# tsinghua-fib-lab/PIML

Measured on AMD Instinct MI355X. Metric: agent-pair force evals/sec + simulated steps/sec, 4096-agent GC scene, higher is better.
Workload: dtype f32

## Files before the change

include/piml_hip_tuning.h:

```cpp
#ifndef PIML_HIP_TUNING_H
#define PIML_HIP_TUNING_H

#include "piml_hip.h"

#ifdef __cplusplus
extern "C" {
#endif

int piml_timer_create(void** event);
int piml_timer_record(void* event, void* stream);
int piml_timer_elapsed_ms(void* start, void* stop, float* ms);
int piml_timer_destroy(void* event);

int piml_trace_begin(void);
int piml_trace_mark(const char* name, void* stream);
int piml_trace_end(char* names, int names_cap, float* us, int us_cap);

int piml_probe_arith(const float* rx, const float* ry, const float* hx, const float* hy,
                     float* dist, float* cosv, int n, void* stream);

long long piml_encoder_split_tiles(long long tiles);
long long piml_encoder_split_tiles_train(long long tiles);
int piml_encoder_products(int split_bf16);
int piml_rowdecoder_products(int split_bf16);
int piml_encoder_dw2(int layer_split);
int piml_encoder_fused_bwd(int on);
int piml_encoder_sums_bwd(int form);
int piml_pinnsf_streams_init(void);

#ifdef __cplusplus
}
#endif
#endif
```

piml_amd/_lib.py:

```python
import ctypes
import os

import torch

_HERE = os.path.dirname(os.path.abspath(__file__))
LIB_PATH = os.environ.get('PIML_LIB') or os.path.join(_HERE, 'libpiml_hip.so')
ABI_VERSION = 35

_lib = None

_i, _f, _p, _z = ctypes.c_int, ctypes.c_float, ctypes.c_void_p, ctypes.c_size_t
_ll = ctypes.c_longlong
_d = ctypes.c_double


class EncoderBranch(ctypes.Structure):
    _fields_ = [('x', _p), ('rows', _ll), ('in_dim', _i), ('k', _i),
                ('w1', _p), ('b1', _p), ('w2', _p), ('b2', _p), ('w3', _p), ('b3', _p),
                ('scale', _f), ('h1', _p), ('h2', _p), ('msgs', _p), ('g_pooled', _p), ('g_msgs', _p),
                ('g2', _p), ('g1', _p), ('g_x', _p), ('partials', _p), ('grads', _p), ('packed', _p), ('relu_mask', _p),
                ('keep_bits', _p), ('drop_state', _p), ('drop_p', _f), ('sum_a', _p), ('sum_b', _p)]


class DecoderBranch(ctypes.Structure):
# ... 98 lines not shown
    'piml_pinnsf_epilogue_ksum_bwd': [_p, _p, _z, _f, _i, _i, _p, _p, _p, _p],
    'piml_pinnsf_epilogue_agentnorm_fwd': [_p, _p, _p, _i, _i, _f, _p, _p],
    'piml_pinnsf_epilogue_ksum_agentnorm_fwd': [_p, _i, _p, _i, _p, _i, _i, _f, _p, _p],
    'piml_pinnsf_epilogue_agentnorm_bwd': [_p, _p, _i, _i, _f, _p, _p],
    'piml_self_features_fwd': [_p, _i, _p, _p, _z, _p, _p],
    'piml_self_features_bwd': [_p, _z, _p, _p, _p, _p],
    'piml_colsum_blocks': [_z, _i],
    'piml_act_bwd_colsum': [_p, _p, _z, _i, _p, _p, _p, _p],
    'piml_sum_leading': [_p, _i, _z, _p, _p],
    'piml_act_bwd_colsum_stage1': [_p, _p, _z, _i, _p, _p, _p, _p],
    'piml_layer_reduce': [_p, _i, _z, _p, _p, _i, _i, _p, _p],
    'piml_scale_ksum_fwd': [_p, _p, _z, _i, _i, _f, _p, _p, _p, _p],
    'piml_ksum_blocks': [_z, _i],
    'piml_scale_ksum_bwd': [_p, _p, _z, _i, _i, _f, _p, _p, _p, _p],
    'piml_dropout_keep_bits': [_p, _ll, _i, _f, _i, _p, _p],
    'piml_timer_create': [ctypes.POINTER(_p)],
    'piml_timer_record': [_p, _p],
    'piml_timer_elapsed_ms': [_p, _p, ctypes.POINTER(_f)],
    'piml_timer_destroy': [_p],
    'piml_trace_begin': [],
    'piml_trace_mark': [ctypes.c_char_p, _p],
    'piml_trace_end': [ctypes.c_char_p, _i, ctypes.POINTER(_f), _i],
    'piml_probe_arith': [_p, _p, _p, _p, _p, _p, _i, _p],
    'piml_encoder_partial_floats': [],
    'piml_encoder_pack_floats': [],
    'piml_encoder_split_tiles': [_ll],
    'piml_encoder_split_tiles_train': [_ll],
    'piml_multi_copy': [ctypes.POINTER(_p), ctypes.POINTER(_p), ctypes.POINTER(_z), _i, _p],
    'piml_rollout_prologue': [_p] * 8 + [_i] * 4 + [_p] * 11 + [_p],
    'piml_rollout_losses_blocks': [_i, _i],
    'piml_rollout_losses': [_p, _p, _ll, _p, _p, _p, _p, _p, _i, _i, _i, _f, _p, _p, _p, _p, _p, _p, _p],
    'piml_rollout_losses_bwd': [_p, _p, _p, _p, _p, _p, _ll, _p, _p],
    'piml_rollout_losses_frames': [_p, _p, _ll, _p, _p, ctypes.POINTER(_p), _i, _p, _i, _i, _i, _f, _f, _f, _p, _p, _p, _p, _p, _p, _p],
    'piml_rollout_losses_frames_bwd': [_p, _p, _p, _p, _f, _f, _p, _p, _p, _ll, _p, _p],
    'piml_collision_pred_loss_blocks': [_ll, _i],
    'piml_collision_pred_loss': [ctypes.POINTER(_p), ctypes.POINTER(_p), _i, _ll, _i, _i, _p, _i, _i, _f, _p, _p, _p, _p, _p],
    'piml_collision_pred_loss_bwd': [_p, _p, _ll, _p, _p],
    'piml_adam_tickets': [],
    'piml_adam_step': [ctypes.POINTER(_p)] * 5 + [ctypes.POINTER(_ll), _i, ctypes.c_double, ctypes.c_double, ctypes.c_double, ctypes.c_double, ctypes.c_double, _p, _p],
    'piml_pointwise_losses_blocks': [_ll, _ll, _i],
    'piml_pointwise_losses': [_p, _p, _ll, _ll, _p, _ll, _f, _p, _i, _p, _p, _p, _p, _p],
    'piml_p2p_alloc': [_z, ctypes.POINTER(_p)],
    'piml_p2p_free': [_p],
    'piml_p2p_export': [_p, _p],
    'piml_p2p_open': [_p, ctypes.POINTER(_p)],
    'piml_p2p_close': [_p],
    'piml_p2p_copy': [_p, _p, _z, _p],
    'piml_allgather_state_p2p': [_p, _z, _i, _i, ctypes.POINTER(_p), ctypes.POINTER(_p), ctypes.c_uint, ctypes.c_uint, _p, _p],
    'piml_encoder_products': [_i],
    'piml_rowdecoder_products': [_i],
    'piml_encoder_dw2': [_i],
    'piml_encoder_fused_bwd': [_i],
    'piml_encoder_sums_bwd': [_i],
    'piml_encoder_pack': [ctypes.POINTER(EncoderBranch), _i, _p],
    'piml_encoder_workgroups': [ctypes.POINTER(EncoderBranch), _i, ctypes.POINTER(_i)],
    'piml_encoder_fwd': [ctypes.POINTER(EncoderBranch), _i, _p],
    'piml_encoder_fwd_packed': [ctypes.POINTER(EncoderBranch), _i, _p],
    'piml_encoder_bwd': [ctypes.POINTER(EncoderBranch), _i, _p],
    'piml_encoder_bwd_acc': [ctypes.POINTER(EncoderBranch), _i, _i, _p],
    'piml_encoder_ksum': [_p, _ll, _i, _p, _p],
    'piml_decoder_pack_floats': [],
    'piml_decoder_partial_floats': [],
    'piml_decoder_workgroups': [_ll],
    'piml_decoder_fwd': [ctypes.POINTER(DecoderBranch), _i, _p, _f, _p, _p],
    'piml_decoder_bwd': [ctypes.POINTER(DecoderBranch), _i, _p, _p, _f, _p, _p],
    'piml_rowdecoder_slots': [_ll],
    'piml_rowdecoder_fwd': [ctypes.POINTER(DecoderBranch), _i, _p],
    'piml_rowdecoder_fwd_packed': [ctypes.POINTER(DecoderBranch), _i, _p],
    'piml_rowdecoder_bwd': [ctypes.POINTER(DecoderBranch), _i, _p],
    'piml_rowdecoder_bwd_acc': [ctypes.POINTER(DecoderBranch), _i, _i, _p],
    'piml_collision_head_pack_floats': [],
    'piml_collision_head_fwd': [_p, _ll, _p, _p, _p, _p, _p, _p, _p],
    'piml_head64_partial_floats': [],
    'piml_head64_slots': [_ll],
    'piml_head64_fwd': [ctypes.POINTER(Head64), _p],
    'piml_head64_bwd': [ctypes.POINTER(Head64), _p],
    'piml_head64_bwd_acc': [ctypes.POINTER(Head64), _i, _p],
    'piml_corrector_partial_floats': [_i],
    'piml_corrector_slots': [_i, _ll, _i],
    'piml_corrector_fwd': [ctypes.POINTER(Corrector), _p],
    'piml_corrector_bwd': [ctypes.POINTER(Corrector), _i, _p],
    'piml_pinnsf_pool_h2_ok': [ctypes.POINTER(EncoderBranch), _i],
    'piml_pinnsf_pool_train_ok': [ctypes.POINTER(EncoderBranch), _i],
    'piml_pinnsf_pool_msgs_ok': [ctypes.POINTER(EncoderBranch), _i],
    'piml_pinnsf_streams_init': [],
    'piml_pinnsf_pack_flush': [],
    'piml_pinnsf_slot_sums_flush': [],
    'piml_pinnsf_pack': [ctypes.POINTER(EncoderBranch), ctypes.POINTER(DecoderBranch), _i, ctypes.POINTER(CollisionHead),
                         _i, _p],
    'piml_pinnsf_fwd': [ctypes.POINTER(EncoderBranch), ctypes.POINTER(DecoderBranch), _i, ctypes.POINTER(CollisionHead),
                        _p, _f, _p, _i, _p],
    'piml_pinnsf_bwd': [ctypes.POINTER(EncoderBranch), ctypes.POINTER(DecoderBranch), _i, _p, _p, _f, _p, _i, _p],
    'piml_comm_available': [],
    'piml_comm_unique_id': [_p],
    'piml_comm_init': [ctypes.POINTER(_p), _i, _i, _p],
    'piml_comm_destroy': [_p],
    'piml_allgather_state': [_p, _p, _z, _p, _p],
    'piml_reducescatter_grad': [_p, _p, _p, _z, _p],
    'piml_allreduce_sum': [_p, _p, _z, _p],
    'piml_relfeat_fwd_self': [_p, _p, _p, _p, _i, _p, _p, _p, _i, _i, _i, _i, _i, _i, _i, _f, _f, _f, _f, _p, _p, _p, _p, _p, _p, _p],
    'piml_relfeat_bwd_self': [_p, _p, _p, _p, _p, _p, _i, _p, _i, _i, _i, _i, _i, _i, _p, _p, _p, _p],
    'piml_relfeat_fwd_tick': [_p, _p, _p, _p, _i, _p, _p, _i, _i, _i, _i, _i, _i, _i, _f, _f, _f, _f,
                              _p, _p, _p, _i, _p, _p, _p, _p],
    'piml_relfeat_self_fwd': [_p, _p, _p, _p, _i, _i, _i, _i, _i, _i, _f, _f, _f, _f, _p, _p, _p, _p, _p, _p, _p],
    'piml_relfeat_self_fwd_part': [_i, _p, _p, _p, _p, _i, _i, _i, _i, _i, _i, _f, _f, _f, _f, _p, _p, _p, _p, _p, _p, _p],
    'piml_relfeat_self_bwd': [_p, _p, _p, _p, _p, _p, _p, _i, _i, _i, _i, _i, _p, _p, _p, _p],
# ... 157 lines not shown
```

piml_amd/csrc/decoder.hip:

```cpp
#include <cstdlib>
#include <type_traits>

#include "common.hpp"
#include "pack.hpp"
#include "reduce.hpp"
#include "stages.hpp"
#include "x3.hpp"
#include "../../include/piml_hip.h"

namespace piml {

typedef float f32x16 __attribute__((ext_vector_type(16)));

constexpr int DEC_SLAB = 32;

struct DecArgs {
    piml_decoder_branch br[2];
    int nbr;
    const float* self_features;
    float tau;
    float* acc;
    const float* g_pred;
    float* g_self;
    int wg_split;
    int pool_h2;
};

#ifdef PIML_DEC_STAMPS
__device__ unsigned long long g_dec_stamps[1024 * 16];
#define DEC_STAMP(i, wait)                                                                         \
    do {                                                                                           \
        __builtin_amdgcn_sched_barrier(0);                                                         \
        if (wait) asm volatile("s_waitcnt vmcnt(0) lgkmcnt(0)" ::: "memory");                      \
        if (threadIdx.x == 0 && blockIdx.x < 1024) g_dec_stamps[blockIdx.x * 16 + (i)] = __builtin_amdgcn_s_memtime(); \
        __builtin_amdgcn_sched_barrier(0);                                                         \
    } while (0)
#else
#define DEC_STAMP(i, wait)
#endif

__device__ __forceinline__ f32x16 dmfma(float a, float b, f32x16 c) {
    return __builtin_amdgcn_mfma_f32_32x32x2f32(a, b, c, 0, 0, 0);
}
__device__ __forceinline__ int dfeat0(int blk, int q, int h) { return 32 * blk + 8 * q + 4 * h; }

__global__ __launch_bounds__(256) void dec_pack_kernel(DecArgs A) {
    const int b = blockIdx.y;
    const piml_decoder_branch J = b ? A.br[1] : A.br[0];
    const int e = blockIdx.x * 256 + threadIdx.x;
    if (e < DEC_PACK) J.packed[e] = dec_pack_value(J, e);
}

__device__ __forceinline__ void dec_pool_body(const piml_decoder_branch& J, long long bx) {
    const long long t = bx * 256 + threadIdx.x;
    if (t >= J.agents * (DH / 4)) return;
    const long long a = t / (DH / 4);
    const int c = (int)(t % (DH / 4));
    const float4* p = reinterpret_cast<const float4*>(J.msgs) + a * J.k * (DH / 4) + c;
    float4 s = make_float4(0.f, 0.f, 0.f, 0.f);
    for (int i = 0; i < J.k; ++i) {
        const float4 v = p[(size_t)i * (DH / 4)];
        s.x += v.x; s.y += v.y; s.z += v.z; s.w += v.w;
    }
    reinterpret_cast<float4*>(J.pooled)[t] = s;
}

__global__ __launch_bounds__(256) void dec_pool_kernel(DecArgs A) {
    dec_pool_body(blockIdx.y ? A.br[1] : A.br[0], blockIdx.x);
}

constexpr int POOL_ROWS = 10;

template <bool POOL, bool SPLIT = false, bool ROWS = false>
__device__ __forceinline__ void dec_fwd_body(const DecArgs& A, long long tile, int split_branch = 0) {
    constexpr int NB = SPLIT ? 1 : 2;
    __shared__ float part1[NB][2][2][16][64];
    __shared__ float part2[NB][2][2][16][64];
    __shared__ float part3[NB][2][2][32];
    __shared__ float poolx[POOL ? NB : 1][POOL ? 4 : 1][POOL ? 16 : 1][64];
    const int lane = threadIdx.x & 63, wave = uniform((int)(threadIdx.x >> 6));
    const int j = lane & 31, h = lane >> 5;
    const int b = SPLIT ? split_branch : wave >> 2, ob = (wave >> 1) & 1, kh = wave & 1;
    const int bi = SPLIT ? 0 : b;
    const bool active = b < A.nbr;
    const piml_decoder_branch J = b ? A.br[1] : A.br[0];
    const long long agent = tile * 32 + j;
    const bool valid = active && agent < J.agents;
    const float4* PK = reinterpret_cast<const float4*>(J.packed);
    const float* bias = J.packed + DP_B;
    float4 w2f[4], w3f[4], w1f[2][4], b2v[4];
// ... 167 lines not shown
#pragma unroll
            for (int q = 0; q < 4; ++q)
                *reinterpret_cast<float4*>(o + dfeat0(kh, q, h)) = make_float4(y[4 * q], y[4 * q + 1], y[4 * q + 2], y[4 * q + 3]);
        }
        f32x16 a3;
#pragma unroll
        for (int r = 0; r < 16; ++r) a3[r] = 0.f;
        if (h == 0 && kh == 0) { a3[0] = b3x; a3[1] = b3y; }
#pragma unroll
        for (int q = 0; q < 4; ++q) {
            const float4 w = w3f[q];
            a3 = dmfma(w.x, y[4 * q + 0], a3);
            a3 = dmfma(w.y, y[4 * q + 1], a3);
            a3 = dmfma(w.z, y[4 * q + 2], a3);
            a3 = dmfma(w.w, y[4 * q + 3], a3);
        }
        if (h == 0) { part3[bi][kh][0][j] = a3[0]; part3[bi][kh][1][j] = a3[1]; }
        if (SPLIT && !POOL && !ROWS) DEC_STAMP(7, true);
    }
    __syncthreads();
    if (SPLIT && !POOL && !ROWS) DEC_STAMP(8, false);
    if (ROWS) {
        if ((wave & 3) == 0 && h == 0 && agent < J.agents)
            reinterpret_cast<float2*>(J.pred)[agent] = make_float2(part3[0][0][0][j] + part3[0][1][0][j],
                                                                   part3[0][0][1][j] + part3[0][1][1][j]);
        return;
    }
    if (wave == 0 && h == 0 && agent < A.br[0].agents) {
        float ax = part3[0][0][0][j] + part3[0][1][0][j], ay = part3[0][0][1][j] + part3[0][1][1][j];
        if (A.self_features && b == 0) {
            const float dx = sfv[0], dy = sfv[1], vx = sfv[2], vy = sfv[3], v0 = sfv[4];
            float t = norm2(dx, dy);
            t = (t == 0.f) ? t + 0.1f : t;
            ax += (v0 * (dx / t) - vx) / A.tau;
            ay += (v0 * (dy / t) - vy) / A.tau;
        }
        if (SPLIT) {
            if (A.nbr > 1) {
                atomicAdd(A.acc + 2 * agent, ax);
                atomicAdd(A.acc + 2 * agent + 1, ay);
            } else {
                reinterpret_cast<float2*>(A.acc)[agent] = make_float2(ax, ay);
            }
        } else {
            if (A.nbr > 1) { ax += part3[1][0][0][j] + part3[1][1][0][j]; ay += part3[1][0][1][j] + part3[1][1][1][j]; }
            reinterpret_cast<float2*>(A.acc)[agent] = make_float2(ax, ay);
        }
    }
    if (SPLIT && !POOL && !ROWS) DEC_STAMP(9, true);
}

__global__ __launch_bounds__(512) void dec_fwd_kernel(DecArgs A) { dec_fwd_body<false>(A, blockIdx.x); }

template <bool ROWS = false, bool SPLIT = false>
__device__ __forceinline__ void dec_bwd_dx_body(const DecArgs& A, long long tile, int rows_branch = 0, float* keep_g2 = nullptr,
                                                float* keep_g1 = nullptr) {
    constexpr int NB = (ROWS || SPLIT) ? 1 : 2;
    __shared__ float part[NB][2][2][16][64];
    const int lane = threadIdx.x & 63, wave = uniform((int)(threadIdx.x >> 6));
    const int j = lane & 31, h = lane >> 5;
    const int b = (ROWS || SPLIT) ? rows_branch : wave >> 2, ob = (wave >> 1) & 1, kh = wave & 1, blk = wave & 3;
    const int bi = (ROWS || SPLIT) ? 0 : b;
    const bool active = b < A.nbr;
    const piml_decoder_branch J = b ? A.br[1] : A.br[0];
    const long long agent = tile * 32 + j;
    const bool valid = active && agent < J.agents;
    const float4* PK = reinterpret_cast<const float4*>(J.packed);
    float2 gp = make_float2(0.f, 0.f);
    float4 hv[2][4], t1f[8];
    float sfv[5] = {0.f, 0.f, 0.f, 0.f, 0.f};
    if (active) {
        gp = reinterpret_cast<const float2*>(ROWS ? J.g_pred_rows : A.g_pred)[valid ? agent : 0];
        if (!valid) gp = make_float2(0.f, 0.f);
        float4 gd2[4];
        if (ROWS && J.g_d2) {
#pragma unroll
            for (int q = 0; q < 4; ++q) gd2[q] = *reinterpret_cast<const float4*>(J.g_d2 + (valid ? agent : 0) * DD + dfeat0(kh, q, h));
        }
        if (!ROWS && wave == 0 && b == 0 && A.g_self && A.self_features) {
            const float* sp = A.self_features + (valid ? agent : 0) * 7;
            sfv[0] = sp[0]; sfv[1] = sp[1]; sfv[4] = sp[6];
        }
        const float bg = h ? gp.y : gp.x;
        const float* hp = J.h1 + (valid ? agent : 0) * DD;
#pragma unroll
        for (int o2 = 0; o2 < 2; ++o2)
#pragma unroll
            for (int q = 0; q < 4; ++q) hv[o2][q] = *reinterpret_cast<const float4*>(hp + dfeat0(o2, q, h));
        const float t3f = J.packed[DP_T3 + 64 * kh + lane];
        float4 t2f[4];
#pragma unroll
        for (int q = 0; q < 4; ++q) t2f[q] = PK[DP_T2 / 4 + (ob * 8 + kh * 4 + q) * 64 + lane];
#pragma unroll
        for (int t = 0; t < 8; ++t) t1f[t] = PK[((!ROWS && A.pool_h2 == 2) ? DP_T1F : DP_T1) / 4 + (blk * 8 + t) * 64 + lane];
        __builtin_amdgcn_sched_barrier(0);
        if (SPLIT) { DEC_STAMP(1, false); DEC_STAMP(2, true); }
        f32x16 g2, g1;
#pragma unroll
        for (int r = 0; r < 16; ++r) { g2[r] = 0.f; g1[r] = 0.f; }
        g2 = dmfma(t3f, bg, g2);
        if (ROWS && J.g_d2) {
#pragma unroll
            for (int q = 0; q < 4; ++q) {
                g2[4 * q] += valid ? gd2[q].x : 0.f; g2[4 * q + 1] += valid ? gd2[q].y : 0.f;
                g2[4 * q + 2] += valid ? gd2[q].z : 0.f; g2[4 * q + 3] += valid ? gd2[q].w : 0.f;
            }
        }
        if (SPLIT && keep_g2) {
            if (ob == 0) {
#pragma unroll
                for (int q = 0; q < 4; ++q)
                    *reinterpret_cast<float4*>(keep_g2 + j * DD + dfeat0(kh, q, h)) =
                        valid ? make_float4(g2[4 * q], g2[4 * q + 1], g2[4 * q + 2], g2[4 * q + 3]) : make_float4(0.f, 0.f, 0.f, 0.f);
            }
        } else if (ob == 0 && valid) {
            float* o = J.g_pre2 + agent * DD;
#pragma unroll
            for (int q = 0; q < 4; ++q)
                *reinterpret_cast<float4*>(o + dfeat0(kh, q, h)) = make_float4(g2[4 * q], g2[4 * q + 1], g2[4 * q + 2], g2[4 * q + 3]);
        }
#pragma unroll
        for (int q = 0; q < 4; ++q) {
            const float4 w = t2f[q];
            g1 = dmfma(w.x, g2[4 * q + 0], g1);
            g1 = dmfma(w.y, g2[4 * q + 1], g1);
            g1 = dmfma(w.z, g2[4 * q + 2], g1);
            g1 = dmfma(w.w, g2[4 * q + 3], g1);
        }
#pragma unroll
        for (int r = 0; r < 16; ++r) part[bi][ob][kh][r][lane] = g1[r];
        if (SPLIT) DEC_STAMP(3, true);
    }
    __syncthreads();
    if (SPLIT) DEC_STAMP(4, false);
    if (active) {
    float g1c[2][16];
#pragma unroll
    for (int o2 = 0; o2 < 2; ++o2)
#pragma unroll
        for (int q = 0; q < 4; ++q) {
            const float4 a = hv[o2][q];
            const float m[4] = {a.x, a.y, a.z, a.w};
#pragma unroll
            for (int u = 0; u < 4; ++u) {
                const float v = part[bi][o2][0][4 * q + u][lane] + part[bi][o2][1][4 * q + u][lane];
                g1c[o2][4 * q + u] = (valid && m[u] > 0.f) ? v : 0.f;
            }
        }
    if (SPLIT && keep_g1) {
        if (blk < 2) {
#pragma unroll
            for (int q = 0; q < 4; ++q) {
                const float4 v0 = make_float4(g1c[0][4 * q], g1c[0][4 * q + 1], g1c[0][4 * q + 2], g1c[0][4 * q + 3]);
                const float4 v1 = make_float4(g1c[1][4 * q], g1c[1][4 * q + 1], g1c[1][4 * q + 2], g1c[1][4 * q + 3]);
                if (blk == 0) *reinterpret_cast<float4*>(keep_g1 + j * DD + dfeat0(0, q, h)) = v0;
                else *reinterpret_cast<float4*>(keep_g1 + j * DD + dfeat0(1, q, h)) = v1;
            }
        }
    } else if (blk < 2 && valid) {
        float* o = J.g_pre1 + agent * DD;
#pragma unroll
        for (int q = 0; q < 4; ++q) {
            const float4 v0 = make_float4(g1c[0][4 * q], g1c[0][4 * q + 1], g1c[0][4 * q + 2], g1c[0][4 * q + 3]);
            const float4 v1 = make_float4(g1c[1][4 * q], g1c[1][4 * q + 1], g1c[1][4 * q + 2], g1c[1][4 * q + 3]);
            if (blk == 0) *reinterpret_cast<float4*>(o + dfeat0(0, q, h)) = v0;
            else *reinterpret_cast<float4*>(o + dfeat0(1, q, h)) = v1;
        }
    }
    {
        f32x16 gpool;
#pragma unroll
        for (int r = 0; r < 16; ++r) gpool[r] = 0.f;
#pragma unroll
        for (int bp = 0; bp < 2; ++bp)
#pragma unroll
            for (int q = 0; q < 4; ++q) {
                const float4 w = t1f[bp * 4 + q];
                gpool = dmfma(w.x, g1c[bp][4 * q + 0], gpool);
                gpool = dmfma(w.y, g1c[bp][4 * q + 1], gpool);
                gpool = dmfma(w.z, g1c[bp][4 * q + 2], gpool);
                gpool = dmfma(w.w, g1c[bp][4 * q + 3], gpool);
            }
        if (valid) {
            float* o = J.g_pooled + agent * DH;
#pragma unroll
            for (int q = 0; q < 4; ++q)
                *reinterpret_cast<float4*>(o + dfeat0(blk, q, h)) =
                    make_float4(gpool[4 * q], gpool[4 * q + 1], gpool[4 * q + 2], gpool[4 * q + 3]);
        }
    }
    }
    if (SPLIT) DEC_STAMP(5, true);
    if (!ROWS && wave == 0 && b == 0 && h == 0 && valid && A.g_self && A.self_features) {
        const float dx = sfv[0], dy = sfv[1], v0 = sfv[4], tau = A.tau;
        const float n = norm2(dx, dy);
        const float t = (n == 0.f) ? n + 0.1f : n;
        const float ex = dx / t, ey = dy / t;
        const float gex = gp.x * v0 / tau, gey = gp.y * v0 / tau;
        const float gt = -(gex * dx + gey * dy) / (t * t);
        float gdx = gex / t, gdy = gey / t;
        if (n != 0.f) { gdx += gt * (dx / n); gdy += gt * (dy / n); }
        float* o = A.g_self + agent * 7;
        o[0] = gdx; o[1] = gdy; o[2] = -gp.x / tau; o[3] = -gp.y / tau; o[4] = 0.f; o[5] = 0.f;
        o[6] = (gp.x * ex + gp.y * ey) / tau;
    }
}

__global__ __launch_bounds__(512) void dec_bwd_dx_kernel(DecArgs A) { dec_bwd_dx_body<false>(A, blockIdx.x); }

template <bool ROWS = false>
__device__ __forceinline__ void dec_bwd_dw_body(const DecArgs& A, int b, int p, int w, int lane, long long slab = DEC_SLAB) {
    const piml_decoder_branch J = b ? A.br[1] : A.br[0];
    const long long R = J.agents;
    const long long s0 = (long long)p * slab < R ? (long long)p * slab : R;
    const long long s1e = s0 + slab < R ? s0 + slab : R;
    const float* __restrict__ in1 = ROWS ? J.msgs : J.pooled;
    const float* __restrict__ gpr = ROWS ? J.g_pred_rows : A.g_pred;
    const int i = lane & 31, h = lane >> 5;
    const int mb1 = w >> 2, nb1 = w & 3, mb2 = (w >> 1) & 1, nb2 = w & 1;
    const bool do2 = w < 4, do3 = w == 4 || w == 5;
    f32x16 c1, c2, c3;
#pragma unroll
    for (int r = 0; r < 16; ++r) { c1[r] = 0.f; c2[r] = 0.f; c3[r] = 0.f; }
    float s1 = 0.f, s2 = 0.f, s3 = 0.f;
    constexpr int U = DEC_SLAB / 2;
    for (long long r0 = s0; r0 < s1e || r0 == s0; r0 += DEC_SLAB) {
        const long long r1 = r0 + DEC_SLAB < s1e ? r0 + DEC_SLAB : s1e;
        float a1[U], b1[U], a2[U], b2[U], a3[U], b3[U];
#pragma unroll
        for (int u = 0; u < U; ++u) {
            const long long row = r0 + 2 * u + h;
            const bool ok = row < r1;
            const long long ro = ok ? row : (r0 < R ? r0 : 0);
            a1[u] = J.g_pre1[ro * DD + 32 * mb1 + i];
            b1[u] = in1[ro * DH + 32 * nb1 + i];
            a2[u] = do2 ? J.g_pre2[ro * DD + 32 * mb2 + i] : 0.f;
            b2[u] = do2 ? J.h1[ro * DD + 32 * nb2 + i] : 0.f;
            a3[u] = (do3 && i < 2) ? gpr[ro * 2 + i] : 0.f;
            b3[u] = do3 ? J.d2[ro * DD + 32 * nb2 + i] : 0.f;
        }
#pragma unroll
        for (int u = 0; u < U; ++u) {
            const bool ok = r0 + 2 * u + h < r1;
            const float x1 = ok ? a1[u] : 0.f, x2 = ok ? a2[u] : 0.f, x3 = ok ? a3[u] : 0.f;
            c1 = dmfma(x1, b1[u], c1);
            if (do2) c2 = dmfma(x2, b2[u], c2);
            if (do3) c3 = dmfma(x3, b3[u], c3);
            s1 += x1; s2 += x2; s3 += x3;
        }
    }
    float* P = J.partials + (size_t)p * DEC_PART;
#pragma unroll
    for (int r = 0; r < 16; ++r) {
        const int ri = (r & 3) + 8 * (r >> 2) + 4 * h;
        P[(size_t)(32 * mb1 + ri) * DH + 32 * nb1 + i] = c1[r];
        if (do2) P[DD * DH + (32 * mb2 + ri) * DD + 32 * nb2 + i] = c2[r];
        if (do3 && ri < 2) P[DD * DH + DD * DD + ri * DD + 32 * nb2 + i] = c3[r];
    }
    s1 += __shfl_xor(s1, 32, 64);
    s2 += __shfl_xor(s2, 32, 64);
    s3 += __shfl_xor(s3, 32, 64);
    float* Pb = P + DD * DH + DD * DD + 2 * DD;
    if (h == 0) {
        if (nb1 == 0) Pb[32 * mb1 + i] = s1;
        if (do2 && nb2 == 0) Pb[DD + 32 * mb2 + i] = s2;
        if (w == 4 && i < 8) Pb[2 * DD + i] = i < 2 ? s3 : 0.f;
    }
}

__device__ __forceinline__ void dec_bwd_dw_body4(const DecArgs& A, int b, int p, int w, int lane, const float* keep_g2, const float* keep_g1) {
    const piml_decoder_branch J = b ? A.br[1] : A.br[0];
    const long long R = J.agents;
    const long long s0 = (long long)p * DEC_SLAB < R ? (long long)p * DEC_SLAB : R;
    const int n = (int)(R - s0 < DEC_SLAB ? R - s0 : DEC_SLAB);
    const long long sb = n > 0 ? s0 : 0;
    const int i = lane & 31, h = lane >> 5;
    const int mb2 = w >> 1, nb2 = w & 1;
    const bool do3 = w < 2;
    constexpr int U = DEC_SLAB / 2;
    const float* __restrict__ pooled0 = J.pooled + sb * DH + 32 * w + i;
    const float* __restrict__ h10 = J.h1 + sb * DD + 32 * nb2 + i;
    const float* __restrict__ d20 = J.d2 + sb * DD + 32 * nb2 + i;
    const float* __restrict__ gp0 = A.g_pred + sb * 2 + (i & 1);
    const float* kg1 = keep_g1 + h * DD + i;
    const float* kg2 = keep_g2 + h * DD + 32 * mb2 + i;
    float a1a[U], a1b[U], b1[U], a2[U], b2[U], a3[U], b3[U];
#pragma unroll
    for (int u = 0; u < U; ++u) {
        a1a[u] = kg1[2 * u * DD];
        a1b[u] = kg1[2 * u * DD + 32];
        a2[u] = kg2[2 * u * DD];
        a3[u] = 0.f; b3[u] = 0.f;
    }
    if (n == DEC_SLAB) {
        const float* pb = pooled0 + h * DH;
        const float* hb = h10 + h * DD;
#pragma unroll
        for (int u = 0; u < U; ++u) { b1[u] = pb[2 * u * DH]; b2[u] = hb[2 * u * DD]; }
        if (do3) {
            const float* db = d20 + h * DD;
            const float* gb = gp0 + h * 2;
#pragma unroll
            for (int u = 0; u < U; ++u) { b3[u] = db[2 * u * DD]; a3[u] = gb[4 * u]; }
        }
    } else {
#pragma unroll
        for (int u = 0; u < U; ++u) {
            const int rc = 2 * u + h < n ? 2 * u + h : 0;
            b1[u] = pooled0[rc * DH]; b2[u] = h10[rc * DD];
        }
        if (do3) {
#pragma unroll
            for (int u = 0; u < U; ++u) {
                const int rc = 2 * u + h < n ? 2 * u + h : 0;
                b3[u] = d20[rc * DD]; a3[u] = gp0[rc * 2];
            }
        }
    }
    DEC_STAMP(8, false);
    DEC_STAMP(9, true);
    f32x16 c1a, c1b, c2, c3;
#pragma unroll
    for (int r = 0; r < 16; ++r) { c1a[r] = 0.f; c1b[r] = 0.f; c2[r] = 0.f; c3[r] = 0.f; }
    float s1a = 0.f, s1b = 0.f, s2 = 0.f, s3 = 0.f;
#pragma unroll
    for (int u = 0; u < U; ++u) {
        c1a = dmfma(a1a[u], b1[u], c1a);
        c1b = dmfma(a1b[u], b1[u], c1b);
        c2 = dmfma(a2[u], b2[u], c2);
        s1a += a1a[u]; s1b += a1b[u]; s2 += a2[u];
    }
    if (do3) {
#pragma unroll
        for (int u = 0; u < U; ++u) {
            const float x3 = (i < 2 && 2 * u + h < n) ? a3[u] : 0.f;
            c3 = dmfma(x3, b3[u], c3);
            s3 += x3;
        }
    }
    float* P = J.partials + (size_t)p * DEC_PART;
    DEC_STAMP(10, false);
    {
#ifdef PIML_DEC_STAMPS
        asm volatile("v_mov_b32 %0, %0" : "+v"(c1a[0]));
        DEC_STAMP(11, false);
#endif
    }
    {
        float* P1 = P + (size_t)(4 * h) * DH + 32 * w + i;
        float* P2 = P + DD * DH + (32 * mb2 + 4 * h) * DD + 32 * nb2 + i;
#pragma unroll
        for (int r = 0; r < 16; ++r) {
            const int rr = (r & 3) + 8 * (r >> 2);
            P1[rr * DH] = c1a[r];
            P1[(32 + rr) * DH] = c1b[r];
            P2[rr * DD] = c2[r];
        }
        if (do3 && h == 0) {
            float* P3 = P + DD * DH + DD * DD + 32 * nb2 + i;
            P3[0] = c3[0]; P3[DD] = c3[1];
        }
    }
    s1a += __shfl_xor(s1a, 32, 64);
    s1b += __shfl_xor(s1b, 32, 64);
    s2 += __shfl_xor(s2, 32, 64);
    s3 += __shfl_xor(s3, 32, 64);
    float* Pb = P + DD * DH + DD * DD + 2 * DD;
    if (h == 0) {
        if (w == 0) { Pb[i] = s1a; Pb[32 + i] = s1b; }
        if (nb2 == 0) Pb[DD + 32 * mb2 + i] = s2;
        if (w == 0 && i < 8) Pb[2 * DD + i] = i < 2 ? s3 : 0.f;
    }
    DEC_STAMP(12, false);
    DEC_STAMP(13, true);
}

__global__ __launch_bounds__(256) void dec_bwd_split_kernel(DecArgs A) {
    const int bx = blockIdx.x;
    const int b = A.nbr > 1 ? (bx & 1) : 0;
    const long long tile = A.nbr > 1 ? (bx >> 1) : bx;
    __shared__ __align__(16) float keep[2][32 * DD];
    DEC_STAMP(0, false);
    dec_bwd_dx_body<false, true>(A, tile, b, keep[0], keep[1]);
    DEC_STAMP(6, false);
    __syncthreads();
    DEC_STAMP(7, false);
    dec_bwd_dw_body4(A, b, (int)tile, uniform((int)(threadIdx.x >> 6)), threadIdx.x & 63, keep[0], keep[1]);
}

__global__ __launch_bounds__(512) void dec_bwd_dw_kernel(DecArgs A) {
    const int lane = threadIdx.x & 63, w = uniform((int)(threadIdx.x >> 6));
    const int b = (A.nbr > 1 && (int)blockIdx.x >= A.wg_split) ? 1 : 0;
    dec_bwd_dw_body<false>(A, b, (int)blockIdx.x - (b ? A.wg_split : 0), w, lane);
}

__global__ __launch_bounds__(512) void dec_bwd_kernel(DecArgs A) {
    dec_bwd_dx_body<false>(A, blockIdx.x);
    __threadfence_block();
    __syncthreads();
    const int lane = threadIdx.x & 63, w = uniform((int)(threadIdx.x >> 6));
    for (int b = 0; b < A.nbr; ++b) dec_bwd_dw_body<false>(A, b, (int)blockIdx.x, w, lane);
}

__global__ __launch_bounds__(256) void rowdec_fwd_kernel(DecArgs A, int tiles0) {
    const int bx = blockIdx.x;
    if (bx < tiles0) dec_fwd_body<false, true, true>(A, bx, 0);
    else dec_fwd_body<false, true, true>(A, bx - tiles0, 1);
}

__global__ __launch_bounds__(256) void rowdec_bwd_dx_kernel(DecArgs A, int tiles0) {
    const int bx = blockIdx.x;
    if (bx < tiles0) dec_bwd_dx_body<true>(A, bx, 0);
    else dec_bwd_dx_body<true>(A, bx - tiles0, 1);
}

template <int NFLOATS>
__device__ __forceinline__ void rowdec_stage(float* lds, const float* __restrict__ src, int tid) {
    constexpr int N4 = NFLOATS / 4, ROUNDS = (N4 + 511) / 512;
    static_assert(NFLOATS % 4 == 0, "float4 granularity");
    const float4* s4 = reinterpret_cast<const float4*>(src);
    float4* d4 = reinterpret_cast<float4*>(lds);
    float4 v[ROUNDS];
#pragma unroll
    for (int r = 0; r < ROUNDS; ++r) {
        const int e = r * 512 + tid;
        v[r] = s4[e < N4 ? e : 0];
    }
#pragma unroll
    for (int r = 0; r < ROUNDS; ++r) {
        const int e = r * 512 + tid;
        if (e < N4) d4[e] = v[r];
    }
}

__global__ __launch_bounds__(512) void rowdec_fwd_big_kernel(DecArgs A, int wg_split) {
    __shared__ __align__(16) float lds[DP_T3];
    const int tid = threadIdx.x, lane = tid & 63, wave = uniform((int)(tid >> 6));
    const int b = (A.nbr > 1 && (int)blockIdx.x >= wg_split) ? 1 : 0;
    const piml_decoder_branch J = b ? A.br[1] : A.br[0];
    const int wg0 = b ? wg_split : 0;
// ... 1116 lines not shown
    const int tiles = (int)((br[0].agents + 31) / 32) * nbr;
    if (g_head_x3) hipLaunchKernelGGL(dec_fwd_head_kernel<true>, dim3((unsigned)(tiles + head_blocks)), dim3(256), head_blocks ? head_lds_bytes(HEAD_LDS_GROUPS_POOL) : 0, s, A, Hd, tiles);
    else hipLaunchKernelGGL(dec_fwd_head_kernel<false>, dim3((unsigned)(tiles + head_blocks)), dim3(256), 0, s, A, Hd, tiles);
    return hipGetLastError();
}

__global__ __launch_bounds__(256) __attribute__((amdgpu_waves_per_eu(2))) void dec_fwd_ph2_kernel(DecArgs A) {
    const int bx = blockIdx.x;
    if (A.nbr > 1) dec_fwd_body<false, true>(A, bx >> 1, bx & 1);
    else dec_fwd_body<false, true>(A, bx, 0);
}

int piml::dec_stage_fwd_ph2(const piml_decoder_branch* br, int nbr, const float* self_features, float tau, float* acc,
                            hipStream_t s) {
    DecArgs A;
    if (!acc) return hipErrorInvalidValue;
    if (int e = dec_fill(A, br, nbr)) return e;
    for (int i = 0; i < nbr; ++i)
        if (!br[i].msgs) return hipErrorInvalidValue;
    A.self_features = self_features;
    A.tau = tau;
    A.acc = acc;
    A.pool_h2 = 1;
    const int tiles = (int)((br[0].agents + 31) / 32) * nbr;
    hipLaunchKernelGGL(dec_fwd_ph2_kernel, dim3((unsigned)tiles), dim3(256), 0, s, A);
    return hipGetLastError();
}

int piml::dec_stage_fwd(const piml_decoder_branch* br, int nbr, const float* self_features, float tau, float* acc,
                        hipStream_t s) {
    DecArgs A;
    if (!acc) return hipErrorInvalidValue;
    if (int e = dec_fill(A, br, nbr)) return e;
    A.self_features = self_features;
    A.tau = tau;
    A.acc = acc;
    const unsigned tiles = (unsigned)((br[0].agents + 31) / 32);
    hipLaunchKernelGGL(dec_fwd_kernel, dim3(tiles), dim3(512), 0, s, A);
    return hipGetLastError();
}

int piml::dec_stage_bwd_dx(const piml_decoder_branch* br, int nbr, const float* g_pred, const float* self_features,
                           float tau, float* g_self, hipStream_t s) {
    DecArgs A;
    if (int e = dec_fill_bwd(A, br, nbr, g_pred)) return e;
    A.self_features = self_features;
    A.tau = tau;
    A.g_self = g_self;
    const unsigned tiles = (unsigned)((br[0].agents + 31) / 32);
    hipLaunchKernelGGL(dec_bwd_dx_kernel, dim3(tiles), dim3(512), 0, s, A);
    return hipGetLastError();
}

int piml::dec_stage_bwd_fused(const piml_decoder_branch* br, int nbr, const float* g_pred, const float* self_features,
                              float tau, float* g_self, hipStream_t s, bool sums) {
    DecArgs A;
    if (int e = dec_fill_bwd(A, br, nbr, g_pred)) return e;
    A.self_features = self_features;
    A.tau = tau;
    A.g_self = g_self;
    if (sums) {
        for (int i = 0; i < nbr; ++i)
            if (!br[i].fold_w3) return hipErrorInvalidValue;
        A.pool_h2 = 2;
    }
    static_assert(DEC_SLAB == 32, "the dW slab of a workgroup is its dX tile");
    const unsigned tiles = (unsigned)((br[0].agents + 31) / 32);
    static const bool whole = getenv("PIML_DEC_BWD_SPLIT") && atoi(getenv("PIML_DEC_BWD_SPLIT")) == 0;
    if (whole && !sums) hipLaunchKernelGGL(dec_bwd_kernel, dim3(tiles), dim3(512), 0, s, A);
    else hipLaunchKernelGGL(dec_bwd_split_kernel, dim3(tiles * (unsigned)nbr), dim3(256), 0, s, A);
    return hipGetLastError();
}

int piml::dec_stage_bwd_dw(const piml_decoder_branch* br, int nbr, const float* g_pred, bool reduce, hipStream_t s) {
    DecArgs A;
    if (int e = dec_fill_bwd(A, br, nbr, g_pred)) return e;
    const int per = dec_dw_workgroups(br[0].agents);
    A.wg_split = per;
    hipLaunchKernelGGL(dec_bwd_dw_kernel, dim3(per * nbr), dim3(512), 0, s, A);
    if (reduce)
        hipLaunchKernelGGL(dec_reduce_kernel, dim3((DEC_PART / 4 + 15) / 16, nbr), dim3(256), 0, s, A, per, DEC_PART / 4);
    return hipGetLastError();
}

static int head_check(const piml_collision_head* h) {
    if (!h || h->rows < 0) return hipErrorInvalidValue;
    if (h->rows > 0 && (!h->msgs || !h->w1 || !h->b1 || !h->w2 || !h->b2 || !h->packed || !h->out)) return hipErrorInvalidValue;
    return hipSuccess;
}

int piml::head_stage_pack(const piml_collision_head* h, hipStream_t s) {
    if (!h || !h->w1 || !h->b1 || !h->w2 || !h->b2 || !h->packed) return hipErrorInvalidValue;
    hipLaunchKernelGGL(head_pack_kernel, dim3((HEAD_PACK + 255) / 256), dim3(256), 0, s, *h);
    return hipGetLastError();
}

int piml::head_stage_fwd(const piml_collision_head* h, hipStream_t s) {
    if (int e = head_check(h)) return e;
    if (h->rows == 0) return hipSuccess;
    const long long tiles = (h->rows + 31) / 32;
    if (g_head_x3) hipLaunchKernelGGL(head_fwd_kernel<true>, dim3((unsigned)((tiles + 3) / 4)), dim3(256), 0, s, h->msgs, h->rows, h->packed, h->out);
    else hipLaunchKernelGGL(head_fwd_kernel<false>, dim3((unsigned)((tiles + 3) / 4)), dim3(256), 0, s, h->msgs, h->rows, h->packed, h->out);
    return hipGetLastError();
}

PIML_API int piml_decoder_fwd(const piml_decoder_branch* br, int nbr, const float* self_features, float tau,
                              float* acc, void* stream) {
    hipStream_t s = as_stream(stream);
    if (int e = dec_stage_pack(br, nbr, s)) return e;
    if (int e = dec_stage_pool(br, nbr, s)) return e;
    return dec_stage_fwd(br, nbr, self_features, tau, acc, s);
}

PIML_API int piml_decoder_bwd(const piml_decoder_branch* br, int nbr, const float* g_pred, const float* self_features,
                              float tau, float* g_self, void* stream) {
    hipStream_t s = as_stream(stream);
    if (int e = dec_stage_bwd_dx(br, nbr, g_pred, self_features, tau, g_self, s)) return e;
    return dec_stage_bwd_dw(br, nbr, g_pred, true, s);
}

static long long rowdec_slab(long long rows) {
    long long slab = (rows + 255) / 256;
    slab = (slab + DEC_SLAB - 1) / DEC_SLAB * DEC_SLAB;
// ... 139 lines not shown
```

Before: 221.5 billion.

## Add helper waves that overlap decoder backward dW with the dX chain

Adds a 512-thread decoder backward kernel, now the default. Four extra helper waves prefetch the dW operands (pooled, h1, d2, g_pred) while the four chain waves compute dX. The helpers compute the g2 and g3 dW products as soon as the barrier passes, then spin on an LDS counter until g1 is ready before doing the g1 products. The aim is to hide the global load latency and the serial dW work behind the dX chain, at the cost of doubled threads per workgroup, higher register pressure and a spin-wait with a custom barrier.

Result: no change. 221.8 billion, median of 6 (+0.1%).

```diff
diff --git a/include/piml_hip_tuning.h b/include/piml_hip_tuning.h
--- a/include/piml_hip_tuning.h
+++ b/include/piml_hip_tuning.h
@@ -26,6 +26,7 @@
 int piml_encoder_dw2(int layer_split);
 int piml_encoder_fused_bwd(int on);
 int piml_encoder_sums_bwd(int form);
+int piml_decoder_bwd_form(int form);
 int piml_pinnsf_streams_init(void);
 
 #ifdef __cplusplus
diff --git a/piml_amd/_lib.py b/piml_amd/_lib.py
--- a/piml_amd/_lib.py
+++ b/piml_amd/_lib.py
@@ -174,6 +174,7 @@
     'piml_encoder_dw2': [_i],
     'piml_encoder_fused_bwd': [_i],
     'piml_encoder_sums_bwd': [_i],
+    'piml_decoder_bwd_form': [_i],
     'piml_encoder_pack': [ctypes.POINTER(EncoderBranch), _i, _p],
     'piml_encoder_workgroups': [ctypes.POINTER(EncoderBranch), _i, ctypes.POINTER(_i)],
     'piml_encoder_fwd': [ctypes.POINTER(EncoderBranch), _i, _p],
diff --git a/piml_amd/csrc/decoder.hip b/piml_amd/csrc/decoder.hip
--- a/piml_amd/csrc/decoder.hip
+++ b/piml_amd/csrc/decoder.hip
@@ -28,14 +28,16 @@
 
 #ifdef PIML_DEC_STAMPS
 __device__ unsigned long long g_dec_stamps[1024 * 16];
-#define DEC_STAMP(i, wait)                                                                         \
+#define DEC_STAMP_AT(i, wait, t)                                                                   \
     do {                                                                                           \
         __builtin_amdgcn_sched_barrier(0);                                                         \
         if (wait) asm volatile("s_waitcnt vmcnt(0) lgkmcnt(0)" ::: "memory");                      \
-        if (threadIdx.x == 0 && blockIdx.x < 1024) g_dec_stamps[blockIdx.x * 16 + (i)] = __builtin_amdgcn_s_memtime(); \
+        if (threadIdx.x == (t) && blockIdx.x < 1024) g_dec_stamps[blockIdx.x * 16 + (i)] = __builtin_amdgcn_s_memtime(); \
         __builtin_amdgcn_sched_barrier(0);                                                         \
     } while (0)
+#define DEC_STAMP(i, wait) DEC_STAMP_AT(i, wait, 0)
 #else
+#define DEC_STAMP_AT(i, wait, t)
 #define DEC_STAMP(i, wait)
 #endif
 
@@ -309,16 +311,17 @@
 
 __global__ __launch_bounds__(512) void dec_fwd_kernel(DecArgs A) { dec_fwd_body<false>(A, blockIdx.x); }
 
-template <bool ROWS = false, bool SPLIT = false>
+template <bool ROWS = false, bool SPLIT = false, bool HELP = false>
 __device__ __forceinline__ void dec_bwd_dx_body(const DecArgs& A, long long tile, int rows_branch = 0, float* keep_g2 = nullptr,
-                                                float* keep_g1 = nullptr) {
+                                                float* keep_g1 = nullptr, int* g1_ready = nullptr) {
+    static_assert(!HELP || (SPLIT && !ROWS), "the helper waves serve the (tile, branch) form");
     constexpr int NB = (ROWS || SPLIT) ? 1 : 2;
     __shared__ float part[NB][2][2][16][64];
     const int lane = threadIdx.x & 63, wave = uniform((int)(threadIdx.x >> 6));
     const int j = lane & 31, h = lane >> 5;
     const int b = (ROWS || SPLIT) ? rows_branch : wave >> 2, ob = (wave >> 1) & 1, kh = wave & 1, blk = wave & 3;
     const int bi = (ROWS || SPLIT) ? 0 : b;
-    const bool active = b < A.nbr;
+    const bool active = b < A.nbr, chain = !HELP || wave < 4;
     const piml_decoder_branch J = b ? A.br[1] : A.br[0];
     const long long agent = tile * 32 + j;
     const bool valid = active && agent < J.agents;
@@ -326,7 +329,7 @@
     float2 gp = make_float2(0.f, 0.f);
     float4 hv[2][4], t1f[8];
     float sfv[5] = {0.f, 0.f, 0.f, 0.f, 0.f};
-    if (active) {
+    if (active && chain) {
         gp = reinterpret_cast<const float2*>(ROWS ? J.g_pred_rows : A.g_pred)[valid ? agent : 0];
         if (!valid) gp = make_float2(0.f, 0.f);
         float4 gd2[4];
@@ -388,10 +391,11 @@
         for (int r = 0; r < 16; ++r) part[bi][ob][kh][r][lane] = g1[r];
         if (SPLIT) DEC_STAMP(3, true);
     }
-    __syncthreads();
+    if (HELP) asm volatile("s_waitcnt lgkmcnt(0)\n\ts_barrier" ::: "memory");
+    else __syncthreads();
     if (SPLIT) DEC_STAMP(4, false);
-    if (active) {
     float g1c[2][16];
+    if (active && chain) {
 #pragma unroll
     for (int o2 = 0; o2 < 2; ++o2)
 #pragma unroll
@@ -424,7 +428,13 @@
             else *reinterpret_cast<float4*>(o + dfeat0(1, q, h)) = v1;
         }
     }
-    {
+    }
+    if (HELP && chain && blk < 2) {
+        __builtin_amdgcn_fence(__ATOMIC_RELEASE, "workgroup");
+        if (lane == 0) __hip_atomic_fetch_add(g1_ready, 1, __ATOMIC_RELAXED, __HIP_MEMORY_SCOPE_WORKGROUP);
+    }
+    if (HELP && !chain) return;
+    if (active && chain) {
         f32x16 gpool;
 #pragma unroll
         for (int r = 0; r < 16; ++r) gpool[r] = 0.f;
@@ -445,7 +455,6 @@
                 *reinterpret_cast<float4*>(o + dfeat0(blk, q, h)) =
                     make_float4(gpool[4 * q], gpool[4 * q + 1], gpool[4 * q + 2], gpool[4 * q + 3]);
         }
-    }
     }
     if (SPLIT) DEC_STAMP(5, true);
     if (!ROWS && wave == 0 && b == 0 && h == 0 && valid && A.g_self && A.self_features) {
@@ -525,84 +534,78 @@
     }
 }
 
-__device__ __forceinline__ void dec_bwd_dw_body4(const DecArgs& A, int b, int p, int w, int lane, const float* keep_g2, const float* keep_g1) {
-    const piml_decoder_branch J = b ? A.br[1] : A.br[0];
-    const long long R = J.agents;
-    const long long s0 = (long long)p * DEC_SLAB < R ? (long long)p * DEC_SLAB : R;
-    const int n = (int)(R - s0 < DEC_SLAB ? R - s0 : DEC_SLAB);
-    const long long sb = n > 0 ? s0 : 0;
+constexpr int DW4_U = DEC_SLAB / 2;
+struct DecDw4 {
+    int n;
+    float b1[DW4_U], b2[DW4_U], b3[DW4_U], a3[DW4_U];
+
+    DecDw4() = default;
+
+    __device__ __forceinline__ DecDw4(const DecArgs& A, const piml_decoder_branch& J, int p, int w, int lane) {
+        const long long R = J.agents;
+        const long long s0 = (long long)p * DEC_SLAB < R ? (long long)p * DEC_SLAB : R;
+        n = (int)(R - s0 < DEC_SLAB ? R - s0 : DEC_SLAB);
+        const long long sb = n > 0 ? s0 : 0;
+        const int i = lane & 31, h = lane >> 5, nb2 = w & 1;
+        const bool do3 = w < 2;
+        const float* __restrict__ pooled0 = J.pooled + sb * DH + 32 * w + i;
+        const float* __restrict__ h10 = J.h1 + sb * DD + 32 * nb2 + i;
+        const float* __restrict__ d20 = J.d2 + sb * DD + 32 * nb2 + i;
+        const float* __restrict__ gp0 = A.g_pred + sb * 2 + (i & 1);
+#pragma unroll
+        for (int u = 0; u < DW4_U; ++u) { a3[u] = 0.f; b3[u] = 0.f; }
+        if (n == DEC_SLAB) {
+            const float* pb = pooled0 + h * DH;
+            const float* hb = h10 + h * DD;
+#pragma unroll
+            for (int u = 0; u < DW4_U; ++u) { b1[u] = pb[2 * u * DH]; b2[u] = hb[2 * u * DD]; }
+            if (do3) {
+                const float* db = d20 + h * DD;
+                const float* gb = gp0 + h * 2;
+#pragma unroll
+                for (int u = 0; u < DW4_U; ++u) { b3[u] = db[2 * u * DD]; a3[u] = gb[4 * u]; }
+            }
+        } else {
+#pragma unroll
+            for (int u = 0; u < DW4_U; ++u) {
+                const int rc = 2 * u + h < n ? 2 * u + h : 0;
+                b1[u] = pooled0[rc * DH]; b2[u] = h10[rc * DD];
+            }
+            if (do3) {
+#pragma unroll
+                for (int u = 0; u < DW4_U; ++u) {
+                    const int rc = 2 * u + h < n ? 2 * u + h : 0;
+                    b3[u] = d20[rc * DD]; a3[u] = gp0[rc * 2];
+                }
+            }
+        }
+    }
+};
+
+__device__ __forceinline__ void dec_dw4_products(const float (&a)[DW4_U], const float (&b)[DW4_U], f32x16& c, float& s) {
+#pragma unroll
+    for (int r = 0; r < 16; ++r) c[r] = 0.f;
+    s = 0.f;
+#pragma unroll
+    for (int u = 0; u < DW4_U; ++u) { c = dmfma(a[u], b[u], c); s += a[u]; }
+}
+
+__device__ __forceinline__ void dec_dw4_a3(const DecDw4& T, int lane, float (&x3)[DW4_U]) {
     const int i = lane & 31, h = lane >> 5;
-    const int mb2 = w >> 1, nb2 = w & 1;
-    const bool do3 = w < 2;
-    constexpr int U = DEC_SLAB / 2;
-    const float* __restrict__ pooled0 = J.pooled + sb * DH + 32 * w + i;
-    const float* __restrict__ h10 = J.h1 + sb * DD + 32 * nb2 + i;
-    const float* __restrict__ d20 = J.d2 + sb * DD + 32 * nb2 + i;
-    const float* __restrict__ gp0 = A.g_pred + sb * 2 + (i & 1);
-    const float* kg1 = keep_g1 + h * DD + i;
-    const float* kg2 = keep_g2 + h * DD + 32 * mb2 + i;
-    float a1a[U], a1b[U], b1[U], a2[U], b2[U], a3[U], b3[U];
-#pragma unroll
-    for (int u = 0; u < U; ++u) {
-        a1a[u] = kg1[2 * u * DD];
-        a1b[u] = kg1[2 * u * DD + 32];
-        a2[u] = kg2[2 * u * DD];
-        a3[u] = 0.f; b3[u] = 0.f;
-    }
-    if (n == DEC_SLAB) {
-        const float* pb = pooled0 + h * DH;
-        const float* hb = h10 + h * DD;
-#pragma unroll
-        for (int u = 0; u < U; ++u) { b1[u] = pb[2 * u * DH]; b2[u] = hb[2 * u * DD]; }
-        if (do3) {
-            const float* db = d20 + h * DD;
-            const float* gb = gp0 + h * 2;
-#pragma unroll
-            for (int u = 0; u < U; ++u) { b3[u] = db[2 * u * DD]; a3[u] = gb[4 * u]; }
-        }
-    } else {
-#pragma unroll
-        for (int u = 0; u < U; ++u) {
-            const int rc = 2 * u + h < n ? 2 * u + h : 0;
-            b1[u] = pooled0[rc * DH]; b2[u] = h10[rc * DD];
-        }
-        if (do3) {
-#pragma unroll
-            for (int u = 0; u < U; ++u) {
-                const int rc = 2 * u + h < n ? 2 * u + h : 0;
-                b3[u] = d20[rc * DD]; a3[u] = gp0[rc * 2];
-            }
-        }
-    }
-    DEC_STAMP(8, false);
-    DEC_STAMP(9, true);
-    f32x16 c1a, c1b, c2, c3;
-#pragma unroll
-    for (int r = 0; r < 16; ++r) { c1a[r] = 0.f; c1b[r] = 0.f; c2[r] = 0.f; c3[r] = 0.f; }
-    float s1a = 0.f, s1b = 0.f, s2 = 0.f, s3 = 0.f;
-#pragma unroll
-    for (int u = 0; u < U; ++u) {
-        c1a = dmfma(a1a[u], b1[u], c1a);
-        c1b = dmfma(a1b[u], b1[u], c1b);
-        c2 = dmfma(a2[u], b2[u], c2);
-        s1a += a1a[u]; s1b += a1b[u]; s2 += a2[u];
-    }
-    if (do3) {
-#pragma unroll
-        for (int u = 0; u < U; ++u) {
-            const float x3 = (i < 2 && 2 * u + h < n) ? a3[u] : 0.f;
-            c3 = dmfma(x3, b3[u], c3);
-            s3 += x3;
-        }
-    }
+#pragma unroll
+    for (int u = 0; u < DW4_U; ++u) x3[u] = (i < 2 && 2 * u + h < T.n) ? T.a3[u] : 0.f;
+}
+
+__device__ __forceinline__ void dec_dw4_lds(const float* keep, int col, int lane, float (&x)[DW4_U]) {
+    const float* k = keep + (lane >> 5) * DD + col + (lane & 31);
+#pragma unroll
+    for (int u = 0; u < DW4_U; ++u) x[u] = k[2 * u * DD];
+}
+
+__device__ __forceinline__ void dec_dw4_store(const piml_decoder_branch& J, int p, int w, int lane, const f32x16& c1a, const f32x16& c1b,
+                                              const f32x16& c2, const f32x16& c3, float s1a, float s1b, float s2, float s3) {
+    const int i = lane & 31, h = lane >> 5, mb2 = w >> 1, nb2 = w & 1;
     float* P = J.partials + (size_t)p * DEC_PART;
-    DEC_STAMP(10, false);
-    {
-#ifdef PIML_DEC_STAMPS
-        asm volatile("v_mov_b32 %0, %0" : "+v"(c1a[0]));
-        DEC_STAMP(11, false);
-#endif
-    }
     {
         float* P1 = P + (size_t)(4 * h) * DH + 32 * w + i;
         float* P2 = P + DD * DH + (32 * mb2 + 4 * h) * DD + 32 * nb2 + i;
@@ -613,7 +616,7 @@
             P1[(32 + rr) * DH] = c1b[r];
             P2[rr * DD] = c2[r];
         }
-        if (do3 && h == 0) {
+        if (w < 2 && h == 0) {
             float* P3 = P + DD * DH + DD * DD + 32 * nb2 + i;
             P3[0] = c3[0]; P3[DD] = c3[1];
         }
@@ -628,6 +631,35 @@
         if (nb2 == 0) Pb[DD + 32 * mb2 + i] = s2;
         if (w == 0 && i < 8) Pb[2 * DD + i] = i < 2 ? s3 : 0.f;
     }
+}
+
+__device__ __forceinline__ void dec_bwd_dw_body4(const DecArgs& A, int b, int p, int w, int lane, const float* keep_g2, const float* keep_g1) {
+    const piml_decoder_branch J = b ? A.br[1] : A.br[0];
+    const bool do3 = w < 2;
+    float a1a[DW4_U], a1b[DW4_U], a2[DW4_U], x3[DW4_U];
+    dec_dw4_lds(keep_g1, 0, lane, a1a);
+    dec_dw4_lds(keep_g1, 32, lane, a1b);
+    dec_dw4_lds(keep_g2, 32 * (w >> 1), lane, a2);
+    const DecDw4 T(A, J, p, w, lane);
+    DEC_STAMP(8, false);
+    DEC_STAMP(9, true);
+    f32x16 c1a, c1b, c2, c3;
+    float s1a, s1b, s2, s3 = 0.f;
+    dec_dw4_products(a1a, T.b1, c1a, s1a);
+    dec_dw4_products(a1b, T.b1, c1b, s1b);
+    dec_dw4_products(a2, T.b2, c2, s2);
+    if (do3) {
+        dec_dw4_a3(T, lane, x3);
+        dec_dw4_products(x3, T.b3, c3, s3);
+    }
+    DEC_STAMP(10, false);
+    {
+#ifdef PIML_DEC_STAMPS
+        asm volatile("v_mov_b32 %0, %0" : "+v"(c1a[0]));
+        DEC_STAMP(11, false);
+#endif
+    }
+    dec_dw4_store(J, p, w, lane, c1a, c1b, c2, c3, s1a, s1b, s2, s3);
     DEC_STAMP(12, false);
     DEC_STAMP(13, true);
 }
@@ -643,6 +675,49 @@
     __syncthreads();
     DEC_STAMP(7, false);
     dec_bwd_dw_body4(A, b, (int)tile, uniform((int)(threadIdx.x >> 6)), threadIdx.x & 63, keep[0], keep[1]);
+}
+
+__global__ __launch_bounds__(512) void dec_bwd_split8_kernel(DecArgs A) {
+    const int bx = blockIdx.x;
+    const int b = A.nbr > 1 ? (bx & 1) : 0;
+    const long long tile = A.nbr > 1 ? (bx >> 1) : bx;
+    __shared__ __align__(16) float keep[2][32 * DD];
+    const int wave = uniform((int)(threadIdx.x >> 6)), lane = threadIdx.x & 63, w = wave & 3;
+    const bool helper = wave >= 4;
+    const piml_decoder_branch J = b ? A.br[1] : A.br[0];
+    __shared__ int g1_ready;
+    DEC_STAMP(0, false);
+    if (threadIdx.x == 0) g1_ready = 0;
+    DecDw4 T;
+    if (helper) T = DecDw4(A, J, (int)tile, w, lane);
+    DEC_STAMP_AT(6, false, 256);
+    dec_bwd_dx_body<false, true, true>(A, tile, b, keep[0], keep[1], &g1_ready);
+    if (!helper) return;
+    DEC_STAMP_AT(7, false, 256);
+    f32x16 c1a, c1b, c2, c3;
+    float s1a, s1b, s2, s3 = 0.f;
+    float a[DW4_U];
+    dec_dw4_lds(keep[0], 32 * (w >> 1), lane, a);
+    dec_dw4_products(a, T.b2, c2, s2);
+    if (w < 2) {
+        dec_dw4_a3(T, lane, a);
+        dec_dw4_products(a, T.b3, c3, s3);
+    }
+    DEC_STAMP_AT(8, false, 256);
+    while (__hip_atomic_load(&g1_ready, __ATOMIC_ACQUIRE, __HIP_MEMORY_SCOPE_WORKGROUP) < 2) __builtin_amdgcn_s_sleep(1);
+    DEC_STAMP_AT(9, false, 256);
+    dec_dw4_lds(keep[1], 0, lane, a);
+    dec_dw4_products(a, T.b1, c1a, s1a);
+    dec_dw4_lds(keep[1], 32, lane, a);
+    dec_dw4_products(a, T.b1, c1b, s1b);
+    DEC_STAMP_AT(10, false, 256);
+#ifdef PIML_DEC_STAMPS
+    asm volatile("v_mov_b32 %0, %0" : "+v"(c1b[0]));
+    DEC_STAMP_AT(11, false, 256);
+#endif
+    dec_dw4_store(J, (int)tile, w, lane, c1a, c1b, c2, c3, s1a, s1b, s2, s3);
+    DEC_STAMP_AT(12, false, 256);
+    DEC_STAMP_AT(13, true, 256);
 }
 
 __global__ __launch_bounds__(512) void dec_bwd_dw_kernel(DecArgs A) {
@@ -1865,6 +1940,14 @@
     return hipGetLastError();
 }
 
+static int g_dec_bwd_form = (getenv("PIML_DEC_BWD_SPLIT") && atoi(getenv("PIML_DEC_BWD_SPLIT")) == 4) ? 4 : 8;
+
+PIML_API int piml_decoder_bwd_form(int form) {
+    const int old = g_dec_bwd_form;
+    if (form == 4 || form == 8) g_dec_bwd_form = form;
+    return old;
+}
+
 int piml::dec_stage_bwd_fused(const piml_decoder_branch* br, int nbr, const float* g_pred, const float* self_features,
                               float tau, float* g_self, hipStream_t s, bool sums) {
     DecArgs A;
@@ -1881,7 +1964,8 @@
     const unsigned tiles = (unsigned)((br[0].agents + 31) / 32);
     static const bool whole = getenv("PIML_DEC_BWD_SPLIT") && atoi(getenv("PIML_DEC_BWD_SPLIT")) == 0;
     if (whole && !sums) hipLaunchKernelGGL(dec_bwd_kernel, dim3(tiles), dim3(512), 0, s, A);
-    else hipLaunchKernelGGL(dec_bwd_split_kernel, dim3(tiles * (unsigned)nbr), dim3(256), 0, s, A);
+    else if (g_dec_bwd_form == 4) hipLaunchKernelGGL(dec_bwd_split_kernel, dim3(tiles * (unsigned)nbr), dim3(256), 0, s, A);
+    else hipLaunchKernelGGL(dec_bwd_split8_kernel, dim3(tiles * (unsigned)nbr), dim3(512), 0, s, A);
     return hipGetLastError();
 }
 
```
